# VojtaHavlicek/AlphaZero-Piskvorky

Hardware: AMD Instinct MI355X
Metric: mcts_node_expansions_per_sec (higher is better)
Workload: dtype f32; 1 GPU; 15x15 / 5-in-a-row self-play, 1024 concurrent games per GPU, 400 sims/move (BASELINE.json configs[3] per-GPU shard), GomokuNet random-init weights, numpy-compatible RNG tapes; board=15, win_length=5, sims_per_move=400, games_per_gpu=1024, engines_per_gpu=4, search_kernel=lock-step (k_trunk, k_fc, k_step per evaluation batch), parallelism=games sharded x1

## Files before the change

alphazero-piskvorky_amd/_capi.py:

```python
import ctypes as C
import os
import subprocess

import numpy as np

_HERE = os.path.dirname(os.path.abspath(__file__))
LIB_PATH = os.environ.get("AZ_ENGINE_LIB") or os.path.join(_HERE, "libaz_engine.so")

STATE_DICT_ORDER = [
    "conv1.weight", "conv1.bias", "conv2.weight", "conv2.bias", "conv3.weight", "conv3.bias",
    "policy_conv.weight", "policy_conv.bias", "policy_fc.weight", "policy_fc.bias",
    "value_conv.weight", "value_conv.bias", "value_fc1.weight", "value_fc1.bias",
    "value_fc2.weight", "value_fc2.bias",
]

AZ_EVAL_NET, AZ_EVAL_SYNTHETIC = 0, 1
AZ_RES_NONE, AZ_RES_X, AZ_RES_O, AZ_RES_DRAW = 0, 1, 2, 3
AZ_AUG_NONE, AZ_AUG_REFERENCE4, AZ_AUG_DIHEDRAL8 = 1, 4, 8
AZ_MODEL_PLAIN, AZ_MODEL_RESNET = 0, 1
AZ_TRUNK_F32, AZ_TRUNK_BF16X3, AZ_TRUNK_F16X2 = 0, 1, 2
AZ_MAX_SIMULATIONS, AZ_DEEP_MAX_SIMULATIONS = 1024, 65534
REUSE_MAX_SIMULATIONS = 1023

EXPORTS = [
    "az_create", "az_create_deep", "az_destroy", "az_last_error", "az_load_weights", "az_load_weights_resnet", "az_net_eval", "az_search", "az_search_batch", "az_search_callback", "az_selfplay",
    "az_selfplay_begin", "az_selfplay_step", "az_selfplay_end", "az_selfplay_games", "az_selfplay_records", "az_selfplay_clear", "az_record_bytes", "az_selfplay_pack", "az_examples_from_packed",
    "az_examples_gather", "az_arena", "az_rules_replay", "az_rng_selfplay_tape", "az_rng_uniforms", "az_set_profiling", "az_set_subtree_reuse", "az_get_counters", "az_get_lanes", "az_get_persistent", "az_set_virtual_loss", "az_set_eval_cache",
    "az_set_trunk_mode", "az_get_trunk_mode", "az_set_leaf_symmetry", "az_emul_split",
    "az_set_start_positions", "az_get_start_positions",
    "az_set_resign", "az_get_resign", "az_selfplay_values", "az_selfplay_pack_values", "az_selfplay_resign_info",
    "az_resign_mix", "az_resign_exempt",
    "az_set_playout_cap", "az_get_playout_cap", "az_playout_cap_full", "az_selfplay_sims", "az_selfplay_export_count",
    "az_set_forced_playouts", "az_get_forced_playouts", "az_forced_prune",
    "az_set_selection", "az_get_selection", "az_selection_tables",
    "az_set_candidates", "az_get_candidates", "az_candidate_mask",
    "az_set_gumbel", "az_get_gumbel", "az_gumbel_schedule", "az_gumbel_target", "az_gumbel_vmix", "az_rng_selfplay_tape_gumbel",
    "az_set_external_evaluator", "az_get_external_evaluator", "az_ext_capacity", "az_ext_stats",
    "az_set_solver", "az_get_solver", "az_last_proof", "az_selfplay_proofs", "az_solver_counts", "az_solver_stops",
    "az_set_win_rule", "az_get_win_rule", "az_rules_winner",
    "az_set_threat_search", "az_get_threat_search", "az_threat_batch", "az_threat_solve", "az_selfplay_threats", "az_threat_stats",
    "az_set_rng", "az_get_rng", "az_rng_philox4x32", "az_rng_log", "az_rng_exp", "az_rng_philox_tape", "az_rng_philox_tape_device",
    "az_set_delta_eval", "az_get_delta_eval", "az_delta_max_tiles", "az_delta_stats", "az_net_eval_delta", "az_delta_lists", "az_delta_lists_full",
    "az_dist_unique_id", "az_dist_init", "az_dist_rank", "az_dist_world", "az_dist_counts", "az_dist_gather_records",
    "az_dist_allreduce_sum", "az_dist_broadcast",
]
AZ_DIST_ID_BYTES = 128


class AzError(RuntimeError):
    pass


class az_config(C.Structure):
    _fields_ = [("board_size", C.c_int32), ("win_length", C.c_int32), ("num_simulations", C.c_int32),
                ("slots", C.c_int32), ("c_puct", C.c_double), ("dirichlet_alpha", C.c_double),
                ("dirichlet_weight", C.c_double), ("eval_kind", C.c_int32), ("device", C.c_int32),
                ("log_table", C.POINTER(C.c_float)), ("model", C.c_int32), ("engines", C.c_int32)]


class az_selfplay_args(C.Structure):
    _fields_ = [("seed0", C.c_uint64), ("num_games", C.c_int32), ("max_plies", C.c_int32),
                ("temperature_table", C.POINTER(C.c_double)), ("noise_tape", C.POINTER(C.c_double)),
                ("u_tape", C.POINTER(C.c_double)), ("tape_stride", C.c_int64)]


class az_counters(C.Structure):
    _fields_ = [("games", C.c_int64), ("plies", C.c_int64), ("records", C.c_int64), ("simulations", C.c_int64),
                ("expansions", C.c_int64), ("root_evals", C.c_int64), ("terminal_hits", C.c_int64),
                ("depth_sum", C.c_int64), ("steps", C.c_int64), ("seconds", C.c_double), ("nn_seconds", C.c_double),
                ("trunk_seconds", C.c_double), ("trunk_launches", C.c_int64), ("trunk_boards", C.c_int64),
                ("step_seconds", C.c_double), ("duplicate_leaves", C.c_int64), ("cache_lookups", C.c_int64),
                ("cache_hits", C.c_int64), ("tape_wait_seconds", C.c_double), ("tape_threads", C.c_int64),
                ("host_cpus", C.c_int64)]

    def as_dict(self):
# ... 104 lines not shown
            L.az_rng_selfplay_tape_gumbel.argtypes = [C.c_uint64, C.c_int, C.c_int, C.c_void_p, C.c_void_p]
        if hasattr(L, "az_set_external_evaluator"):
            L.az_set_external_evaluator.argtypes = [C.c_void_p, C.POINTER(az_ext_evaluator)]
            L.az_get_external_evaluator.argtypes = [C.c_void_p]
            L.az_ext_capacity.argtypes = [C.c_void_p]
            L.az_ext_stats.argtypes = [C.c_void_p, C.POINTER(C.c_int64), C.POINTER(C.c_int64)]
        if hasattr(L, "az_set_solver"):
            L.az_set_solver.argtypes = [C.c_void_p, C.c_int]
            L.az_get_solver.argtypes = [C.c_void_p]
            L.az_last_proof.argtypes = [C.c_void_p, C.c_int, C.c_void_p, C.c_void_p, C.POINTER(C.c_int32)]
            L.az_solver_stops.argtypes = [C.c_void_p, C.POINTER(C.c_int64)]
            L.az_selfplay_proofs.argtypes = [C.c_void_p, C.c_void_p]
            L.az_solver_counts.argtypes = [C.c_int, C.c_void_p, C.c_void_p, C.c_void_p]
        if hasattr(L, "az_set_win_rule"):
            L.az_set_win_rule.argtypes = [C.c_void_p, C.c_int]
            L.az_get_win_rule.argtypes = [C.c_void_p]
            L.az_rules_winner.argtypes = [C.c_void_p, C.c_int, C.c_int, C.c_int]
        if hasattr(L, "az_set_threat_search"):
            L.az_set_threat_search.argtypes = [C.c_void_p, C.c_int, C.c_int]
            L.az_get_threat_search.argtypes = [C.c_void_p, C.POINTER(C.c_int), C.POINTER(C.c_int)]
            L.az_threat_batch.argtypes = [C.c_void_p, C.c_int, C.c_void_p, C.c_void_p, C.c_int, C.c_int] + [C.c_void_p] * 5
            L.az_threat_solve.argtypes = [C.c_void_p, C.c_int, C.c_int, C.c_int, C.c_int, C.c_int, C.c_int] + [C.c_void_p] * 4
            L.az_selfplay_threats.argtypes = [C.c_void_p, C.c_void_p]
            L.az_threat_stats.argtypes = [C.c_void_p] + [C.POINTER(C.c_int64)] * 5
        if hasattr(L, "az_set_delta_eval"):
            L.az_set_delta_eval.argtypes = [C.c_void_p, C.c_int]
            L.az_get_delta_eval.argtypes = [C.c_void_p]
            L.az_delta_max_tiles.argtypes = [C.c_void_p, C.c_int]
            L.az_delta_stats.argtypes = [C.c_void_p] + [C.POINTER(C.c_int64)] * 4 + [C.c_void_p]
            L.az_net_eval_delta.argtypes = [C.c_void_p, C.c_int, C.c_void_p, C.c_int, C.c_int] + [C.c_void_p] * 7
            L.az_delta_lists.argtypes = [C.c_int, C.c_int] + [C.c_void_p] * 5
        if hasattr(L, "az_delta_lists_full"):
            L.az_delta_lists_full.argtypes = [C.c_int] + [C.c_void_p] * 4
        if hasattr(L, "az_set_rng"):
            L.az_set_rng.argtypes = [C.c_void_p, C.c_int]
            L.az_get_rng.argtypes = [C.c_void_p]
            L.az_rng_philox4x32.argtypes = [C.c_void_p, C.c_void_p, C.c_void_p]
            L.az_rng_philox4x32.restype = None
            L.az_rng_log.argtypes = L.az_rng_exp.argtypes = [C.c_double]
            L.az_rng_log.restype = L.az_rng_exp.restype = C.c_double
            L.az_rng_philox_tape.argtypes = [C.c_uint64, C.c_int, C.c_double, C.c_int, C.c_int, C.c_void_p, C.c_void_p]
            L.az_rng_philox_tape_device.argtypes = [C.c_void_p, C.c_uint64, C.c_int, C.c_double, C.c_int, C.c_int, C.c_void_p, C.c_void_p]
        _LIB = L
    return _LIB


def _p(a):
    return None if a is None else a.ctypes.data_as(C.c_void_p)


def _dp(a):
    return None if a is None else a.ctypes.data_as(C.POINTER(C.c_double))


def rng_selfplay_tape(seed, n, alpha=0.3, max_plies=0):
    nn = n * n
    plies = max_plies if 0 < max_plies < nn else nn
    total = sum(nn - m for m in range(plies))
    noise = np.zeros(total, np.float64)
    u = np.zeros(nn, np.float64)
    rc = lib().az_rng_selfplay_tape(int(seed), n, float(alpha), int(max_plies), _p(noise), _p(u))
    if rc:
        raise AzError(f"az_rng_selfplay_tape failed ({rc})")
    return noise, u[:plies]


# ... 865 lines not shown
```

alphazero-piskvorky_amd/csrc/az_delta.h:

```cpp
#pragma once
#include "az_net.h"

constexpr int DELTA_MAX_CHANGED = 8;
constexpr int DELTA_TILES_DEFAULT = 12;
constexpr int DELTA_CNT = 4 + 16;

template <int N>
struct DeltaGeo : NetGeo<N> {
    typedef NetGeo<N> B;
    static constexpr int IMG = 96 * B::CS;
    static constexpr int STRIDE = IMG + B::FROW;
    static constexpr int MAXM = ((B::nn + 15) / 16) * 16;
    static constexpr int C3 = 4;
};

__host__ __device__ inline int delta_dist(int n, int pr, int pc, const unsigned char *changed, int nch)
{
    int best = 255;
    for (int i = 0; i < nch; i++) {
        const int cr = changed[i] / n, cc = changed[i] - cr * n;
        const int dr = pr - 1 - cr < 0 ? cr - (pr - 1) : pr - 1 - cr, dc = pc - 1 - cc < 0 ? cc - (pc - 1) : pc - 1 - cc;
        const int dd = dr > dc ? dr : dc;
        best = dd < best ? dd : best;
    }
    return best;
}
__host__ __device__ inline bool delta_member(int n, int list, int pr, int pc, int dist)
{
    const bool inb = pr >= 1 && pr <= n && pc >= 1 && pc <= n;
    return list < 3 ? (inb && dist <= list + 1) : dist <= list;
}
template <int N>
struct DeltaLists {
    typedef DeltaGeo<N> G;
    unsigned short wpos[3][G::MAXM], cell[3][G::MAXM];
    unsigned short halo[2][G::PP];
    int cnt[5];
    __host__ __device__ int tiles(int l) const { return (cnt[l] + 15) >> 4; }
    __host__ __device__ void put(int list, int at, int pr, int pc)
    {
        const unsigned short pos = (unsigned short)(pr * G::PW + pc);
        if (list < 3) { wpos[list][at] = pos; cell[list][at] = (unsigned short)((pr - 1) * N + (pc - 1)); }
        else halo[list - 3][at] = pos;
    }
    __host__ __device__ void junk(int list, int i)
    {
        const int c = cnt[list], at = c + i;
        if (c > 0 && at < tiles(list) * 16) { wpos[list][at] = wpos[list][c - 1]; cell[list][at] = 0xFFFF; }
    }
};
template <int N>
__host__ __device__ inline void delta_lists_serial(const unsigned char *changed, int nch, DeltaLists<N> &L)
{
    typedef DeltaGeo<N> G;
    for (int l = 0; l < 5; l++) L.cnt[l] = 0;
    for (int p = 0; p < G::PP; p++) {
        const int pr = p / G::PW, pc = p - pr * G::PW;
        const int dist = delta_dist(N, pr, pc, changed, nch);
        for (int l = 0; l < 5; l++)
            if (delta_member(N, l, pr, pc, dist)) L.put(l, L.cnt[l]++, pr, pc);
    }
    for (int l = 0; l < 3; l++)
        for (int i = 0; i < 16; i++) L.junk(l, i);
}
template <int N>
__host__ __device__ inline void delta_full_put(DeltaLists<N> &L, int pr, int pc)
{
    if (pr < 1 || pr > N || pc < 1 || pc > N) return;
    for (int l = 0; l < 3; l++) L.put(l, (pr - 1) * N + (pc - 1), pr, pc);
}
template <int N>
__host__ __device__ inline void delta_full_cnt(DeltaLists<N> &L, int l) { L.cnt[l] = l < 3 ? N * N : 0; }
template <int N>
__host__ __device__ inline void delta_lists_full(DeltaLists<N> &L)
{
    typedef DeltaGeo<N> G;
    for (int p = 0; p < G::PP; p++) delta_full_put<N>(L, p / G::PW, p % G::PW);
    for (int l = 0; l < 5; l++) delta_full_cnt<N>(L, l);
    for (int l = 0; l < 3; l++)
        for (int i = 0; i < 16; i++) L.junk(l, i);
}

#ifdef __HIPCC__
#ifdef AZ_STAMPS
#define AZ_DSTAMP(k) do { if (threadIdx.x == 0 && dbg) dbg[(size_t)blockIdx.x * 16 + (k)] = __builtin_amdgcn_s_memtime(); } while (0)
#define AZ_DSTAMP_VAL(k, v) do { if (threadIdx.x == 0 && dbg) dbg[(size_t)blockIdx.x * 16 + (k)] = (unsigned long long)(v); } while (0)
#else
#define AZ_DSTAMP(k) do { } while (0)
#define AZ_DSTAMP_VAL(k, v) do { } while (0)
#endif

template <class G>
__device__ __forceinline__ void delta_heads(const NetWeights &w, float *__restrict__ frow, const float *out3, const float *hdq_lds,
                                            const unsigned short *cellof, int ncell, int wave, int lane)
{
    if (wave * 32 >= ncell) return;
    const int half = (lane >> 2) & 1;
    const int m = wave * 32 + (lane >> 3) * 4 + (lane & 3);
    float hb[4];
#pragma unroll
    for (int i = 0; i < 4; i++) hb[i] = (half * 4 + i) < 6 ? w.hdb[half * 4 + i] : 0.0f;
    const float4 *ap = reinterpret_cast<const float4 *>(hdq_lds) + (lane & 7);
    const float4 *bp = reinterpret_cast<const float4 *>(out3 + (m < ncell ? m : 0) * OUT3_CM_STRIDE);
    f32x4 acc = f32x4{0.f, 0.f, 0.f, 0.f};
#pragma unroll
    for (int k4 = 0; k4 < 32; k4++) {
        const float4 a = ap[k4 * 8], b = bp[k4];
        acc = __builtin_amdgcn_mfma_f32_4x4x1f32(a.x, b.x, acc, 0, 0, 0);
        acc = __builtin_amdgcn_mfma_f32_4x4x1f32(a.y, b.y, acc, 0, 0, 0);
        acc = __builtin_amdgcn_mfma_f32_4x4x1f32(a.z, b.z, acc, 0, 0, 0);
        acc = __builtin_amdgcn_mfma_f32_4x4x1f32(a.w, b.w, acc, 0, 0, 0);
    }
    if (m < ncell) {
        const int cell = cellof[m];
        if (cell != 0xFFFF) {
#pragma unroll
// ... 54 lines not shown
        float4 *z = reinterpret_cast<float4 *>(lds);
        for (int i = tid; i < (96 * G::CS) / 4; i += G::NW * 64) z[i] = float4{0.f, 0.f, 0.f, 0.f};
    }
    __syncthreads();
    float *inA = lds, *inB = lds + 32 * G::CS;
    if (e_me) inB[e_pos] = 1.0f;
    if (e_op) inB[G::CS + e_pos] = 1.0f;
    __syncthreads();
    conv_layer<G, 4, 32, CONV_OUT_PACKED>(inB, inA, w.c1, w.c1b, wpos, cellof, wave, lane);
    __syncthreads();
    for (int i = tid; i < 3 * G::CS; i += G::NW * 64) inB[i] = 0.0f;
    __syncthreads();
    conv_layer<G, 32, 64, CONV_OUT_PACKED>(inA, inB, w.c2, w.c2b, wpos, cellof, wave, lane);
    __syncthreads();
    float *row = base + ((size_t)b * 2 + par) * DG::STRIDE;
    {
        const float4 *s = reinterpret_cast<const float4 *>(lds);
        float4 *g = reinterpret_cast<float4 *>(row);
        for (int i = tid; i < DG::IMG / 4; i += G::NW * 64) g[i] = s[i];
    }
    conv_layer<G, 64, 128, CONV_OUT3_CM>(inB, lds, w.c3, w.c3b, wpos, cellof, wave, lane);
    __syncthreads();
    trunk_heads<G>(d, w, net_id, row + DG::IMG - (size_t)b * G::FROW, lds, hdq_lds, cellof, b, wave, lane);
    if (tid == 0 && par == 0) cnt[(size_t)b * DELTA_CNT + 3] += 2ull;
}

template <int N>
__global__ __launch_bounds__(NetGeo<N>::NW * 64) void k_trunk_delta(DevState d, NetWeights w, int net_id, float *__restrict__ feat,
                                                                     const float *__restrict__ base, unsigned char *done,
                                                                     unsigned long long *cnt, int max_tiles, unsigned long long *dbg)
{
    typedef DeltaGeo<N> G;
    constexpr int NT = G::NW * 64;
    static_assert(G::G == 1 && NT >= G::PP && NT == 512, "one board per workgroup, one thread per padded position");
    static_assert(G::C3 * 16 * OUT3_CM_STRIDE <= 32 * G::CS, "a chunk's conv3 image fits the dead conv1 image");
    static_assert(G::STRIDE % 4 == 0, "16-byte rows");
    __shared__ __attribute__((aligned(16))) float lds[G::IMG];
    __shared__ __attribute__((aligned(16))) float planes[4 * G::CS];
    __shared__ __attribute__((aligned(16))) float hdq_lds[1024];
    __shared__ DeltaLists<N> L;
    __shared__ unsigned char changed[DELTA_MAX_CHANGED];
    __shared__ int s_nch;
    __shared__ int s_wc[5][5];
    const int b = blockIdx.x;
    if (b >= d.B) return;
    const int tid = threadIdx.x, lane = tid & 63;
    const int wave = __builtin_amdgcn_readfirstlane(tid >> 6);
    AZ_DSTAMP(0);
    AZ_DSTAMP_VAL(14, __builtin_amdgcn_s_memrealtime());
#ifdef AZ_STAMPS
    for (int k = 1; k < 14; k++) AZ_DSTAMP_VAL(k, 0);
#endif
    {
        const int kind = d.leaf_kind[b];
        if (!((kind == LEAF_ROOT || kind == LEAF_EXPAND) && d.s_status[b] == SLOT_ACTIVE && d.s_net[b] == net_id)) {
            if (tid == 0) done[b] = 1;
            return;
        }
    }
    const float2 hq = reinterpret_cast<const float2 *>(w.hdq)[tid];
    const u64 *lf = d.leaf + (size_t)b * 8, *bd = d.board + (size_t)b * 8;
    const int last = d.leaf_last[b];
    int stones = 0;
#pragma unroll
    for (int i = 0; i < 8; i++) stones += __popcll(lf[i]) - __popcll(bd[i]);
    const int par = stones & 1;
    bool e_me = false, e_op = false, e_last = false;
    int e_pos = G::PW + 1;
    if (tid == 0) s_nch = 0;
    for (int i = tid; i < 4 * G::CS; i += NT) planes[i] = 0.0f;
    reinterpret_cast<float2 *>(hdq_lds)[tid] = hq;
    __syncthreads();
    if (tid < G::nn) {
        const int r = tid / N, c = tid - r * N;
        e_pos = (r + 1) * G::PW + (c + 1);
        e_me = (lf[tid >> 6] >> (tid & 63)) & 1ull;
        e_op = (lf[4 + (tid >> 6)] >> (tid & 63)) & 1ull;
        e_last = last == tid;
        const bool x = (bd[tid >> 6] >> (tid & 63)) & 1ull, o = (bd[4 + (tid >> 6)] >> (tid & 63)) & 1ull;
        const bool me_is_x = (d.s_player[b] == 1) != (par == 1);
        if (e_me != (me_is_x ? x : o) || e_op != (me_is_x ? o : x) || e_last) {
            const int k = atomicAdd(&s_nch, 1);
            if (k < DELTA_MAX_CHANGED) changed[k] = (unsigned char)tid;
        }
        if (e_me) planes[e_pos] = 1.0f;
        if (e_op) planes[G::CS + e_pos] = 1.0f;
        if (e_last) planes[2 * G::CS + e_pos] = 1.0f;
    }
    __syncthreads();
    const int nch = s_nch;
    bool full = nch > DELTA_MAX_CHANGED;
    const int pr = tid / G::PW, pc = tid - pr * G::PW;
    int dist = 255;
    if (!full) {
        u64 bal[5] = {0, 0, 0, 0, 0};
        if (wave < 5) {
            const bool in_img = tid < G::PP;
            if (in_img) dist = delta_dist(N, pr, pc, changed, nch);
#pragma unroll
            for (int l = 0; l < 5; l++) {
                bal[l] = __ballot(in_img && delta_member(N, l, pr, pc, dist));
                if (lane == 0) s_wc[wave][l] = __popcll(bal[l]);
            }
        }
        __syncthreads();
        if (wave < 5 && tid < G::PP) {
#pragma unroll
            for (int l = 0; l < 5; l++) {
                if (!((bal[l] >> lane) & 1ull)) continue;
                int at = __popcll(bal[l] & ((1ull << lane) - 1ull));
                for (int v = 0; v < wave; v++) at += s_wc[v][l];
                L.put(l, at, pr, pc);
            }
        }
        if (tid < 5) L.cnt[tid] = s_wc[0][tid] + s_wc[1][tid] + s_wc[2][tid] + s_wc[3][tid] + s_wc[4][tid];
        __syncthreads();
        full = L.tiles(2) > max_tiles;
        if (full) __syncthreads();
    }
    float *inA = lds, *inB = lds + 32 * G::CS;
    if (full) {
        if (tid < G::PP) delta_full_put<N>(L, pr, pc);
        if (tid < 5) delta_full_cnt<N>(L, tid);
        float4 *z = reinterpret_cast<float4 *>(lds);
        for (int i = tid; i < G::IMG / 4; i += NT) z[i] = float4{0.f, 0.f, 0.f, 0.f};
        __syncthreads();
    }
    const int t1 = L.tiles(0), t2 = L.tiles(1), t3 = L.tiles(2);
    AZ_DSTAMP(1);
    AZ_DSTAMP_VAL(13, t3);
    if (tid < 48) L.junk(tid >> 4, tid & 15);
    if (tid == 0) {
        if (full) { done[b] = 0; cnt[(size_t)b * DELTA_CNT + 1] += 1ull; }
        else {
            done[b] = (unsigned char)(1 + t3);
            cnt[(size_t)b * DELTA_CNT + 0] += 1ull;
            cnt[(size_t)b * DELTA_CNT + 2] += (unsigned long long)t3;
            cnt[(size_t)b * DELTA_CNT + 4 + t3] += 1ull;
        }
    }
    constexpr int WR = (G::PP + 63) / 64;
    static_assert(WR * 64 >= G::PP && G::NW == 8, "the rounds reach the longest list; one conv1 plane and two conv2 planes per wave");
    f32x4 w1[WR], w2[2][WR];
    float fr[6];
    f32x4 *l4 = reinterpret_cast<f32x4 *>(lds);
    float *frow = feat + (size_t)b * G::FROW;
    const bool keep = !full && tid < G::PP && delta_member(N, 2, pr, pc, 0) && dist > 3;
    const int fcell = (pr - 1) * N + (pc - 1);
    const int n3 = full ? 0 : L.cnt[3], n4 = full ? 0 : L.cnt[4];
    {
        const float *brow = base + ((size_t)b * 2 + par) * G::STRIDE;
        const f32x4 *g4 = reinterpret_cast<const f32x4 *>(brow);
        const float *bf = brow + G::IMG;
        delta_rounds<0, WR>([&](auto jc) {
            constexpr int j = decltype(jc)::value;
            if (j * 64 + lane < n3) w1[j] = g4[wave * G::CS + L.halo[0][j * 64 + lane]];
        });
        delta_rounds<0, WR>([&](auto jc) {
            constexpr int j = decltype(jc)::value;
            if (j * 64 + lane < n4) {
                const int pos = L.halo[1][j * 64 + lane];
                w2[0][j] = g4[(8 + wave) * G::CS + pos];
                w2[1][j] = g4[(16 + wave) * G::CS + pos];
            }
        });
        if (keep) {
#pragma unroll
            for (int i = 0; i < 6; i++) fr[i] = bf[i * G::nn + fcell];
        }
        delta_rounds<0, WR>([&](auto jc) {
            constexpr int j = decltype(jc)::value;
            if (j * 64 + lane < n3) l4[wave * G::CS + L.halo[0][j * 64 + lane]] = w1[j];
        });
    }
    __syncthreads();
    AZ_DSTAMP(2);
    for (int t0 = 0; t0 < t1; t0 += 4)
        conv_layer<G, 4, 32, CONV_OUT_PACKED, 4>(planes, inA, w.c1, w.c1b, L.wpos[0], L.cell[0], wave, lane, t0, t1 - t0 < 4 ? t1 - t0 : 4);
    delta_rounds<0, WR>([&](auto jc) {
        constexpr int j = decltype(jc)::value;
        if (j * 64 + lane < n4) {
            const int pos = L.halo[1][j * 64 + lane];
            l4[(8 + wave) * G::CS + pos] = w2[0][j];
            l4[(16 + wave) * G::CS + pos] = w2[1][j];
        }
    });
    if (keep) {
#pragma unroll
        for (int i = 0; i < 6; i++) frow[i * G::nn + fcell] = fr[i];
    }
    __syncthreads();
    AZ_DSTAMP(3);
    for (int t0 = 0; t0 < t2;) {
        const int c = t2 - t0;
        if (c > 2) { conv_layer<G, 32, 64, CONV_OUT_PACKED, 4>(inA, inB, w.c2, w.c2b, L.wpos[1], L.cell[1], wave, lane, t0, c < 4 ? c : 4); t0 += 4; }
        else { conv_layer<G, 32, 64, CONV_OUT_PACKED, 2>(inA, inB, w.c2, w.c2b, L.wpos[1], L.cell[1], wave, lane, t0, c); t0 += 2; }
    }
    __syncthreads();
    AZ_DSTAMP(4);
    for (int t0 = 0; t0 < t3; t0 += G::C3) {
        const int c = t3 - t0 < G::C3 ? t3 - t0 : G::C3;
        float *o3 = lds - t0 * 16 * OUT3_CM_STRIDE;
        if (c == 4) conv_layer<G, 64, 128, CONV_OUT3_CM, 4>(inB, o3, w.c3, w.c3b, L.wpos[2], L.cell[2], wave, lane, t0, 4);
        else if (c == 3) conv_layer<G, 64, 128, CONV_OUT3_CM, 3>(inB, o3, w.c3, w.c3b, L.wpos[2], L.cell[2], wave, lane, t0, 3);
        else if (c == 2) conv_layer<G, 64, 128, CONV_OUT3_CM, 2>(inB, o3, w.c3, w.c3b, L.wpos[2], L.cell[2], wave, lane, t0, 2);
        else conv_layer<G, 64, 128, CONV_OUT3_CM, 1>(inB, o3, w.c3, w.c3b, L.wpos[2], L.cell[2], wave, lane, t0, 1);
        __syncthreads();
        AZ_DSTAMP(5 + 2 * (t0 / G::C3));
        delta_heads<G>(w, frow, lds, hdq_lds, L.cell[2] + t0 * 16, c * 16, wave, lane);
        __syncthreads();
        AZ_DSTAMP(6 + 2 * (t0 / G::C3));
        AZ_DSTAMP_VAL(15, __builtin_amdgcn_s_memrealtime());
    }
}
#endif
```

alphazero-piskvorky_amd/csrc/az_engine.hip:

```cpp
#include <hip/hip_runtime.h>
#include <dlfcn.h>
#include <sched.h>

#include <algorithm>
#include <atomic>
#include <chrono>
#include <condition_variable>
#include <cmath>
#include <cstdarg>
#include <cstdio>
#include <cstdlib>
#include <cstring>
#include <mutex>
#include <string>
#include <thread>
#include <vector>

#define AZ_ENGINE_TU 1
#include "../../include/az_engine.h"
#include "az_launch.h"

#include "az_host.h"

static thread_local std::string g_create_error;
// ... 2434 lines not shown
}

extern "C" int az_delta_lists(int n, int count, const uint8_t *changed, uint16_t *wpos, uint16_t *cell, uint16_t *halo, int32_t *cnt)
{
    if (n != 15 || count < 0 || count > DELTA_MAX_CHANGED || (count && !changed) || !wpos || !cell || !halo || !cnt) return AZ_ERR_INVALID;
    for (int i = 0; i < count; i++) if (changed[i] >= 15 * 15) return AZ_ERR_INVALID;
    static DeltaLists<15> L;
    static std::mutex m;
    std::lock_guard<std::mutex> lock(m);
    memset(&L, 0xEE, sizeof L);
    delta_lists_serial<15>(changed, count, L);
    memcpy(wpos, L.wpos, sizeof L.wpos);
    memcpy(cell, L.cell, sizeof L.cell);
    memcpy(halo, L.halo, sizeof L.halo);
    for (int l = 0; l < 5; l++) cnt[l] = L.cnt[l];
    return AZ_OK;
}

extern "C" int az_delta_lists_full(int n, uint16_t *wpos, uint16_t *cell, uint16_t *halo, int32_t *cnt)
{
    if (n != 15 || !wpos || !cell || !halo || !cnt) return AZ_ERR_INVALID;
    static DeltaLists<15> L;
    static std::mutex m;
    std::lock_guard<std::mutex> lock(m);
    memset(&L, 0xEE, sizeof L);
    delta_lists_full<15>(L);
    memcpy(wpos, L.wpos, sizeof L.wpos);
    memcpy(cell, L.cell, sizeof L.cell);
    memcpy(halo, L.halo, sizeof L.halo);
    for (int l = 0; l < 5; l++) cnt[l] = L.cnt[l];
    return AZ_OK;
}

extern "C" int az_net_eval_delta(az_engine *e, int slot, const uint8_t *root, int root_player, int count, const uint8_t *boards,
                                 const uint8_t *players, const int16_t *lasts, float *logits, float *policy, float *value, int32_t *path)
{
    if (!e || slot < 0 || slot > 1 || count < 0 || !root || !boards || !players || !lasts || (root_player != 1 && root_player != 2))
        return fail(e, AZ_ERR_INVALID, "az_net_eval_delta: bad argument");
    if (!e->net[slot].loaded) return fail(e, AZ_ERR_NO_WEIGHTS, "weights slot %d not loaded", slot);
    if (e->run.open) return fail(e, AZ_ERR_STATE, "az_net_eval_delta: a self-play episode is open on this engine");
    if (!e->ops->trunk_delta || e->cfg.model != AZ_MODEL_PLAIN || e->cfg.eval_kind != AZ_EVAL_NET)
        return fail(e, AZ_ERR_INVALID, "az_net_eval_delta: no delta evaluation for this board size or net");
    DEVICE_GUARD(e);
    int rc = ensure_delta_buffers(e);
    if (rc) return rc;
    const Lane &L = e->lanes[0];
    const DeltaRoot dr{root, root_player, path};
    return eval_positions(e, "az_net_eval_delta", slot, count, boards, players, lasts, logits, policy, value, &dr, [&](LaunchCtx &lc, int) {
        lc.delta_base = (float *)L.delta_base.p;
        lc.delta_done = (unsigned char *)L.delta_done.p;
        lc.delta_cnt = (unsigned long long *)L.delta_cnt.p;
        lc.delta_tiles = e->delta_tiles;
        e->ops->trunk_base(lc, slot);
        e->ops->trunk_delta(lc, slot);
    });
}

extern "C" int az_selfplay_proofs(az_engine *e, int8_t *roots)
{
    if (!e || !e->have_episode) return fail(e, AZ_ERR_STATE, "no episode has been run");
    if (!roots) return fail(e, AZ_ERR_INVALID, "az_selfplay_proofs: null buffer");
    if (!e->episode_solver || !e->rec_proof.p) return fail(e, AZ_ERR_STATE, "az_selfplay_proofs: the episode ran without the solver");
    DEVICE_GUARD(e);
    return read_record_array(e, e->rec_proof, roots);
}

// ... 1012 lines not shown
```

include/az_engine.h:

```cpp
#ifndef AZ_ENGINE_H
#define AZ_ENGINE_H

#include <stdint.h>

#ifdef __cplusplus
extern "C" {
#endif

typedef struct az_engine az_engine;

typedef enum {
    AZ_OK = 0,
    AZ_ERR_INVALID = -1,
    AZ_ERR_NO_DEVICE = -2,
    AZ_ERR_HIP = -3,
    AZ_ERR_ILLEGAL_MOVE = -4,
    AZ_ERR_NO_WEIGHTS = -5,
    AZ_ERR_STATE = -6
} az_status;

enum { AZ_EVAL_NET = 0, AZ_EVAL_SYNTHETIC = 1 };
enum { AZ_RES_NONE = 0, AZ_RES_X = 1, AZ_RES_O = 2, AZ_RES_DRAW = 3 };
enum { AZ_AUG_REFERENCE4 = 4, AZ_AUG_DIHEDRAL8 = 8, AZ_AUG_NONE = 1 };
enum { AZ_TRUNK_F32 = 0, AZ_TRUNK_BF16X3 = 1, AZ_TRUNK_F16X2 = 2 };
// ... 132 lines not shown
             int32_t *nply);

int az_rules_replay(az_engine *e, int games, int max_len, const int16_t *actions, uint8_t *term_before, uint8_t *boards,
                    int32_t *players, int32_t *results, int32_t *first_illegal);

int az_rng_selfplay_tape(uint64_t seed, int board_size, double alpha, int max_plies, double *noise, double *u);
int az_rng_uniforms(uint64_t seed, int count, double *u);
int az_rng_selfplay_tape_gumbel(uint64_t seed, int board_size, int max_plies, double *noise, double *u);

enum { AZ_RNG_NUMPY = 0, AZ_RNG_PHILOX = 1 };
enum { AZ_TAPE_DIRICHLET = 0, AZ_TAPE_GUMBEL = 1 };
#define AZ_RNG_PHILOX_ATTEMPTS 64
int az_set_rng(az_engine *e, int mode);
int az_get_rng(const az_engine *e);
void az_rng_philox4x32(const uint32_t ctr[4], const uint32_t key[2], uint32_t out[4]);
double az_rng_log(double x);
double az_rng_exp(double x);
int az_rng_philox_tape(uint64_t seed, int board_size, double alpha, int max_plies, int kind, double *noise, double *u);
int az_rng_philox_tape_device(az_engine *e, uint64_t seed0, int games, double alpha, int max_plies, int kind, double *noise_out,
                              double *u_out);

int az_set_subtree_reuse(az_engine *e, int on);

int az_set_virtual_loss(az_engine *e, int leaves);

int az_set_eval_cache(az_engine *e, int64_t entries);

int az_set_delta_eval(az_engine *e, int on);
int az_get_delta_eval(const az_engine *e);
int az_delta_max_tiles(az_engine *e, int tiles);
int az_delta_stats(const az_engine *e, int64_t *delta, int64_t *full, int64_t *tiles, int64_t *base, int64_t *by_tiles);
int az_delta_lists(int n, int count, const uint8_t *changed, uint16_t *wpos, uint16_t *cell, uint16_t *halo, int32_t *cnt);
int az_delta_lists_full(int n, uint16_t *wpos, uint16_t *cell, uint16_t *halo, int32_t *cnt);
int az_net_eval_delta(az_engine *e, int slot, const uint8_t *root, int root_player, int count, const uint8_t *boards,
                      const uint8_t *players, const int16_t *lasts, float *logits, float *policy, float *value, int32_t *path);

int az_set_leaf_symmetry(az_engine *e, int on);

int az_set_start_positions(az_engine *e, int count, const uint8_t *boards ,
                           const uint8_t *players, const int16_t *lasts, int64_t first);
int az_get_start_positions(const az_engine *e);

enum { AZ_RULE_FREESTYLE = 0, AZ_RULE_EXACT = 1 };
int az_set_win_rule(az_engine *e, int rule);
int az_get_win_rule(const az_engine *e);
int az_rules_winner(const uint8_t *board, int n, int k, int rule);

uint32_t az_resign_mix(uint32_t x);
int az_resign_exempt(uint32_t key, int playout_permille);
int az_set_resign(az_engine *e, double threshold, int min_ply, int playout_permille);
int az_get_resign(const az_engine *e, double *threshold, int *min_ply, int *playout_permille);
int az_selfplay_values(az_engine *e, float *values);
int az_selfplay_pack_values(az_engine *e, float *values_dev);
int az_selfplay_resign_info(az_engine *e, int32_t *cross_ply, uint8_t *exempt);

int az_playout_cap_full(uint32_t key, int ply, int full_permille);
int az_set_playout_cap(az_engine *e, int fast_sims, int full_permille, int export_full_only);
int az_get_playout_cap(const az_engine *e, int *fast_sims, int *full_permille, int *export_full_only);
int az_selfplay_sims(az_engine *e, int32_t *sims);
int az_selfplay_export_count(az_engine *e, int64_t *records);

int az_set_forced_playouts(az_engine *e, double k, int prune);
int az_get_forced_playouts(const az_engine *e, double *k, int *prune);
int64_t az_forced_prune(double k, double c_puct, int count, const int32_t *visits, const double *W, const float *prior, int32_t *out);

int az_set_selection(az_engine *e, int on, double fpu, double fpu_root, double cpuct_base, double cpuct_factor);
// ... 49 lines not shown
```

Baseline: 6.606 million node-expansions/s.

## Restructure delta-eval kernel prologue to cut barriers and shared-memory atomics

The delta evaluation kernel now finds changed cells with wave-uniform bit arithmetic (readfirstlane plus per-lane popcount/ctz) instead of a shared-memory atomic scan. It also folds list counting into a single vectorized read of per-wave counts, which removes several __syncthreads. Conv1 now runs over the conv3 tile list instead of copying halo values, conv1/conv2 weights are prefetched before the early exit, and statistics counters use relaxed atomics. The goal is lower per-leaf prologue latency and less synchronisation. In exchange conv1 may compute more tiles, and the list-building logic is more intricate.

```diff
diff --git a/alphazero-piskvorky_amd/_capi.py b/alphazero-piskvorky_amd/_capi.py
--- a/alphazero-piskvorky_amd/_capi.py
+++ b/alphazero-piskvorky_amd/_capi.py
@@ -41,6 +41,7 @@
     "az_set_threat_search", "az_get_threat_search", "az_threat_batch", "az_threat_solve", "az_selfplay_threats", "az_threat_stats",
     "az_set_rng", "az_get_rng", "az_rng_philox4x32", "az_rng_log", "az_rng_exp", "az_rng_philox_tape", "az_rng_philox_tape_device",
     "az_set_delta_eval", "az_get_delta_eval", "az_delta_max_tiles", "az_delta_stats", "az_net_eval_delta", "az_delta_lists", "az_delta_lists_full",
+    "az_delta_changed",
     "az_dist_unique_id", "az_dist_init", "az_dist_rank", "az_dist_world", "az_dist_counts", "az_dist_gather_records",
     "az_dist_allreduce_sum", "az_dist_broadcast",
 ]
@@ -211,6 +212,8 @@
             L.az_delta_lists.argtypes = [C.c_int, C.c_int] + [C.c_void_p] * 5
         if hasattr(L, "az_delta_lists_full"):
             L.az_delta_lists_full.argtypes = [C.c_int] + [C.c_void_p] * 4
+        if hasattr(L, "az_delta_changed"):
+            L.az_delta_changed.argtypes = [C.c_int, C.c_void_p, C.c_void_p, C.c_int, C.c_int] + [C.c_void_p] * 3
         if hasattr(L, "az_set_rng"):
             L.az_set_rng.argtypes = [C.c_void_p, C.c_int]
             L.az_get_rng.argtypes = [C.c_void_p]
diff --git a/alphazero-piskvorky_amd/csrc/az_delta.h b/alphazero-piskvorky_amd/csrc/az_delta.h
--- a/alphazero-piskvorky_amd/csrc/az_delta.h
+++ b/alphazero-piskvorky_amd/csrc/az_delta.h
@@ -48,6 +48,11 @@
         const int c = cnt[list], at = c + i;
         if (c > 0 && at < tiles(list) * 16) { wpos[list][at] = wpos[list][c - 1]; cell[list][at] = 0xFFFF; }
     }
+    __host__ __device__ void junk_at(int list, int c, int i, int pos)
+    {
+        const int at = c + i;
+        if (i >= 0 && i < 16 && at < ((c + 15) >> 4) * 16) { wpos[list][at] = (unsigned short)pos; cell[list][at] = 0xFFFF; }
+    }
 };
 template <int N>
 __host__ __device__ inline void delta_lists_serial(const unsigned char *changed, int nch, DeltaLists<N> &L)
@@ -81,7 +86,47 @@
         for (int i = 0; i < 16; i++) L.junk(l, i);
 }
 
+template <int N>
+__host__ __device__ inline __attribute__((always_inline)) int delta_changed(const u64 *leaf, const u64 *board, int player, int last, int k, int *count, int *parity)
+{
+    static_assert(N * N > 192 && N * N <= 256, "four words of cells, the last one in part");
+    int stones = 0;
+#pragma unroll
+    for (int i = 0; i < 8; i++) stones += __builtin_popcountll(leaf[i]) - __builtin_popcountll(board[i]);
+    const int par = stones & 1;
+    const bool me_is_x = (player == 1) != (par == 1);
+    u64 v = 0;
+    int total = 0, wi = 0, kk = 0;
+#pragma unroll
+    for (int i = 0; i < 4; i++) {
+        const u64 bme = me_is_x ? board[i] : board[4 + i], bop = me_is_x ? board[4 + i] : board[i];
+        u64 dw = (leaf[i] ^ bme) | (leaf[4 + i] ^ bop);
+        if (last >= 0 && last < N * N && (last >> 6) == i) dw |= 1ull << (last & 63);
+        if (i == 3 && N * N < 256) dw &= (1ull << ((N * N) & 63)) - 1ull;
+        const int c = __builtin_popcountll(dw);
+        if (k >= total && k < total + c) { v = dw; wi = i; kk = k - total; }
+        total += c;
+    }
+#pragma unroll
+    for (int j = 0; j < DELTA_MAX_CHANGED - 1; j++)
+        if (j < kk) v &= v - 1ull;
+    *count = total;
+    *parity = par;
+    return (k >= 0 && k < total && k < DELTA_MAX_CHANGED && v) ? wi * 64 + __builtin_ctzll(v) : 0xFF;
+}
+
 #ifdef __HIPCC__
+__device__ __forceinline__ void delta_count(unsigned long long *p, unsigned long long v)
+{
+    (void)__hip_atomic_fetch_add(p, v, __ATOMIC_RELAXED, __HIP_MEMORY_SCOPE_AGENT);
+}
+
+__device__ __forceinline__ u64 delta_uniform(u64 v)
+{
+    const unsigned lo = __builtin_amdgcn_readfirstlane((unsigned)v), hi = __builtin_amdgcn_readfirstlane((unsigned)(v >> 32));
+    return ((u64)hi << 32) | lo;
+}
+
 #ifdef AZ_STAMPS
 #define AZ_DSTAMP(k) do { if (threadIdx.x == 0 && dbg) dbg[(size_t)blockIdx.x * 16 + (k)] = __builtin_amdgcn_s_memtime(); } while (0)
 #define AZ_DSTAMP_VAL(k, v) do { if (threadIdx.x == 0 && dbg) dbg[(size_t)blockIdx.x * 16 + (k)] = (unsigned long long)(v); } while (0)
@@ -202,16 +247,14 @@
 {
     typedef DeltaGeo<N> G;
     constexpr int NT = G::NW * 64;
-    static_assert(G::G == 1 && NT >= G::PP && NT == 512, "one board per workgroup, one thread per padded position");
+    static_assert(G::G == 1 && NT >= G::CS && NT == 512, "one board per workgroup, one thread per padded position");
     static_assert(G::C3 * 16 * OUT3_CM_STRIDE <= 32 * G::CS, "a chunk's conv3 image fits the dead conv1 image");
     static_assert(G::STRIDE % 4 == 0, "16-byte rows");
     __shared__ __attribute__((aligned(16))) float lds[G::IMG];
     __shared__ __attribute__((aligned(16))) float planes[4 * G::CS];
     __shared__ __attribute__((aligned(16))) float hdq_lds[1024];
     __shared__ DeltaLists<N> L;
-    __shared__ unsigned char changed[DELTA_MAX_CHANGED];
-    __shared__ int s_nch;
-    __shared__ int s_wc[5][5];
+    __shared__ __attribute__((aligned(16))) int s_wc[5][4];
     const int b = blockIdx.x;
     if (b >= d.B) return;
     const int tid = threadIdx.x, lane = tid & 63;
@@ -221,111 +264,113 @@
 #ifdef AZ_STAMPS
     for (int k = 1; k < 14; k++) AZ_DSTAMP_VAL(k, 0);
 #endif
-    {
-        const int kind = d.leaf_kind[b];
-        if (!((kind == LEAF_ROOT || kind == LEAF_EXPAND) && d.s_status[b] == SLOT_ACTIVE && d.s_net[b] == net_id)) {
-            if (tid == 0) done[b] = 1;
-            return;
-        }
-    }
+    const int kind = d.leaf_kind[b], status = d.s_status[b], snet = d.s_net[b], last = d.leaf_last[b], player = d.s_player[b];
+    u64 lf[8], bd[8];
+#pragma unroll
+    for (int i = 0; i < 8; i++) { lf[i] = delta_uniform(d.leaf[(size_t)b * 8 + i]); bd[i] = delta_uniform(d.board[(size_t)b * 8 + i]); }
     const float2 hq = reinterpret_cast<const float2 *>(w.hdq)[tid];
-    const u64 *lf = d.leaf + (size_t)b * 8, *bd = d.board + (size_t)b * 8;
-    const int last = d.leaf_last[b];
-    int stones = 0;
-#pragma unroll
-    for (int i = 0; i < 8; i++) stones += __popcll(lf[i]) - __popcll(bd[i]);
-    const int par = stones & 1;
-    bool e_me = false, e_op = false, e_last = false;
-    int e_pos = G::PW + 1;
-    if (tid == 0) s_nch = 0;
-    for (int i = tid; i < 4 * G::CS; i += NT) planes[i] = 0.0f;
-    reinterpret_cast<float2 *>(hdq_lds)[tid] = hq;
-    __syncthreads();
-    if (tid < G::nn) {
-        const int r = tid / N, c = tid - r * N;
-        e_pos = (r + 1) * G::PW + (c + 1);
-        e_me = (lf[tid >> 6] >> (tid & 63)) & 1ull;
-        e_op = (lf[4 + (tid >> 6)] >> (tid & 63)) & 1ull;
-        e_last = last == tid;
-        const bool x = (bd[tid >> 6] >> (tid & 63)) & 1ull, o = (bd[4 + (tid >> 6)] >> (tid & 63)) & 1ull;
-        const bool me_is_x = (d.s_player[b] == 1) != (par == 1);
-        if (e_me != (me_is_x ? x : o) || e_op != (me_is_x ? o : x) || e_last) {
-            const int k = atomicAdd(&s_nch, 1);
-            if (k < DELTA_MAX_CHANGED) changed[k] = (unsigned char)tid;
-        }
-        if (e_me) planes[e_pos] = 1.0f;
-        if (e_op) planes[G::CS + e_pos] = 1.0f;
-        if (e_last) planes[2 * G::CS + e_pos] = 1.0f;
-    }
-    __syncthreads();
-    const int nch = s_nch;
+    const ConvPre<4> pre1 = conv_prefetch<G, 4, 32>(w.c1, wave, lane);
+    if (!((kind == LEAF_ROOT || kind == LEAF_EXPAND) && status == SLOT_ACTIVE && snet == net_id)) {
+        if (tid == 0) done[b] = 1;
+        return;
+    }
+    int ch[DELTA_MAX_CHANGED], par, nch;
+    {
+        const int mine = delta_changed<N>(lf, bd, player, last, lane & (DELTA_MAX_CHANGED - 1), &nch, &par);
+#pragma unroll
+        for (int i = 0; i < DELTA_MAX_CHANGED; i++) ch[i] = __builtin_amdgcn_readlane(mine, i);
+    }
     bool full = nch > DELTA_MAX_CHANGED;
     const int pr = tid / G::PW, pc = tid - pr * G::PW;
+    const bool in_img = tid < G::PP, inb = in_img && pr >= 1 && pr <= N && pc >= 1 && pc <= N;
+    const int fcell = (pr - 1) * N + (pc - 1);
+    f32x4 *l4 = reinterpret_cast<f32x4 *>(lds);
+    if (tid < G::CS) {
+        const int cp = inb ? fcell : 0, wi = cp >> 6;
+        const u64 me = wi == 0 ? lf[0] : wi == 1 ? lf[1] : wi == 2 ? lf[2] : lf[3];
+        const u64 op = wi == 0 ? lf[4] : wi == 1 ? lf[5] : wi == 2 ? lf[6] : lf[7];
+        planes[tid] = inb && ((me >> (cp & 63)) & 1ull) ? 1.0f : 0.0f;
+        planes[G::CS + tid] = inb && ((op >> (cp & 63)) & 1ull) ? 1.0f : 0.0f;
+        planes[2 * G::CS + tid] = inb && last == cp ? 1.0f : 0.0f;
+        planes[3 * G::CS + tid] = 0.0f;
+    }
     int dist = 255;
+    u64 bal[4] = {0, 0, 0, 0};
+    if (!full && wave < 5) {
+        if (in_img) {
+#pragma unroll
+            for (int i = 0; i < DELTA_MAX_CHANGED; i++) {
+                if (i < nch) {
+                    const int cr = ch[i] / N, cc = ch[i] - cr * N;
+                    const int dr = pr - 1 - cr < 0 ? cr - (pr - 1) : pr - 1 - cr, dc = pc - 1 - cc < 0 ? cc - (pc - 1) : pc - 1 - cc;
+                    const int dd = dr > dc ? dr : dc;
+                    dist = dd < dist ? dd : dist;
+                }
+            }
+        }
+#pragma unroll
+        for (int l = 0; l < 4; l++) {
+            bal[l] = __ballot(in_img && delta_member(N, l < 3 ? l : 4, pr, pc, dist));
+            if (lane == 0) s_wc[wave][l] = __popcll(bal[l]);
+        }
+        if (in_img && !inb && dist <= 3) {
+#pragma unroll
+            for (int k = 0; k < 8; k++) l4[k * G::CS + tid] = f32x4{0.f, 0.f, 0.f, 0.f};
+        }
+    }
+    __syncthreads();
+    int c[4] = {G::nn, G::nn, G::nn, 0}, front[4] = {0, 0, 0, 0};
     if (!full) {
-        u64 bal[5] = {0, 0, 0, 0, 0};
-        if (wave < 5) {
-            const bool in_img = tid < G::PP;
-            if (in_img) dist = delta_dist(N, pr, pc, changed, nch);
-#pragma unroll
-            for (int l = 0; l < 5; l++) {
-                bal[l] = __ballot(in_img && delta_member(N, l, pr, pc, dist));
-                if (lane == 0) s_wc[wave][l] = __popcll(bal[l]);
+        c[0] = c[1] = c[2] = 0;
+#pragma unroll
+        for (int v = 0; v < 5; v++) {
+            const int4 r = reinterpret_cast<const int4 *>(&s_wc[0][0])[v];
+            const int rv[4] = {r.x, r.y, r.z, r.w};
+#pragma unroll
+            for (int l = 0; l < 4; l++) { c[l] += rv[l]; front[l] += v < wave ? rv[l] : 0; }
+        }
+        full = ((c[2] + 15) >> 4) > max_tiles;
+        if (full) { c[0] = c[1] = c[2] = G::nn; c[3] = 0; }
+    }
+    if (!full) {
+        if (wave < 5 && in_img) {
+#pragma unroll
+            for (int l = 0; l < 4; l++) {
+                if ((bal[l] >> lane) & 1ull) L.put(l < 3 ? l : 4, front[l] + __popcll(bal[l] & ((1ull << lane) - 1ull)), pr, pc);
+                if (l < 3 && bal[l] && front[l] + __popcll(bal[l]) == c[l])
+                    L.junk_at(l, c[l], lane, wave * 64 + 63 - __builtin_clzll(bal[l]));
             }
         }
-        __syncthreads();
-        if (wave < 5 && tid < G::PP) {
-#pragma unroll
-            for (int l = 0; l < 5; l++) {
-                if (!((bal[l] >> lane) & 1ull)) continue;
-                int at = __popcll(bal[l] & ((1ull << lane) - 1ull));
-                for (int v = 0; v < wave; v++) at += s_wc[v][l];
-                L.put(l, at, pr, pc);
-            }
-        }
-        if (tid < 5) L.cnt[tid] = s_wc[0][tid] + s_wc[1][tid] + s_wc[2][tid] + s_wc[3][tid] + s_wc[4][tid];
-        __syncthreads();
-        full = L.tiles(2) > max_tiles;
-        if (full) __syncthreads();
-    }
-    float *inA = lds, *inB = lds + 32 * G::CS;
-    if (full) {
-        if (tid < G::PP) delta_full_put<N>(L, pr, pc);
-        if (tid < 5) delta_full_cnt<N>(L, tid);
-        float4 *z = reinterpret_cast<float4 *>(lds);
-        for (int i = tid; i < G::IMG / 4; i += NT) z[i] = float4{0.f, 0.f, 0.f, 0.f};
-        __syncthreads();
-    }
-    const int t1 = L.tiles(0), t2 = L.tiles(1), t3 = L.tiles(2);
+    } else {
+        if (in_img) delta_full_put<N>(L, pr, pc);
+#pragma unroll
+        for (int l = 0; l < 3; l++) L.junk_at(l, G::nn, tid, N * G::PW + N);
+        for (int i = tid; i < G::IMG / 4; i += NT) l4[i] = f32x4{0.f, 0.f, 0.f, 0.f};
+    }
+    __syncthreads();
+    const int t2 = (c[1] + 15) >> 4, t3 = (c[2] + 15) >> 4, n4 = c[3];
     AZ_DSTAMP(1);
-    AZ_DSTAMP_VAL(13, t3);
-    if (tid < 48) L.junk(tid >> 4, tid & 15);
+    AZ_DSTAMP_VAL(13, t3 | (t2 << 8));
     if (tid == 0) {
-        if (full) { done[b] = 0; cnt[(size_t)b * DELTA_CNT + 1] += 1ull; }
+        unsigned long long *cb = cnt + (size_t)b * DELTA_CNT;
+        if (full) { done[b] = 0; delta_count(cb + 1, 1ull); }
         else {
             done[b] = (unsigned char)(1 + t3);
-            cnt[(size_t)b * DELTA_CNT + 0] += 1ull;
-            cnt[(size_t)b * DELTA_CNT + 2] += (unsigned long long)t3;
-            cnt[(size_t)b * DELTA_CNT + 4 + t3] += 1ull;
+            delta_count(cb + 0, 1ull);
+            delta_count(cb + 2, (unsigned long long)t3);
+            delta_count(cb + 4 + t3, 1ull);
         }
     }
     constexpr int WR = (G::PP + 63) / 64;
-    static_assert(WR * 64 >= G::PP && G::NW == 8, "the rounds reach the longest list; one conv1 plane and two conv2 planes per wave");
-    f32x4 w1[WR], w2[2][WR];
+    static_assert(WR * 64 >= G::PP && G::NW == 8, "the rounds reach the longest list; two conv2 planes per wave");
+    f32x4 w2[2][WR];
     float fr[6];
-    f32x4 *l4 = reinterpret_cast<f32x4 *>(lds);
     float *frow = feat + (size_t)b * G::FROW;
-    const bool keep = !full && tid < G::PP && delta_member(N, 2, pr, pc, 0) && dist > 3;
-    const int fcell = (pr - 1) * N + (pc - 1);
-    const int n3 = full ? 0 : L.cnt[3], n4 = full ? 0 : L.cnt[4];
+    const bool keep = !full && inb && dist > 3;
     {
         const float *brow = base + ((size_t)b * 2 + par) * G::STRIDE;
         const f32x4 *g4 = reinterpret_cast<const f32x4 *>(brow);
         const float *bf = brow + G::IMG;
-        delta_rounds<0, WR>([&](auto jc) {
-            constexpr int j = decltype(jc)::value;
-            if (j * 64 + lane < n3) w1[j] = g4[wave * G::CS + L.halo[0][j * 64 + lane]];
-        });
         delta_rounds<0, WR>([&](auto jc) {
             constexpr int j = decltype(jc)::value;
             if (j * 64 + lane < n4) {
@@ -338,15 +383,14 @@
 #pragma unroll
             for (int i = 0; i < 6; i++) fr[i] = bf[i * G::nn + fcell];
         }
-        delta_rounds<0, WR>([&](auto jc) {
-            constexpr int j = decltype(jc)::value;
-            if (j * 64 + lane < n3) l4[wave * G::CS + L.halo[0][j * 64 + lane]] = w1[j];
-        });
-    }
-    __syncthreads();
+    }
+    const ConvPre<32> pre2 = conv_prefetch<G, 32, 64>(w.c2, wave, lane);
     AZ_DSTAMP(2);
-    for (int t0 = 0; t0 < t1; t0 += 4)
-        conv_layer<G, 4, 32, CONV_OUT_PACKED, 4>(planes, inA, w.c1, w.c1b, L.wpos[0], L.cell[0], wave, lane, t0, t1 - t0 < 4 ? t1 - t0 : 4);
+    float *inA = lds, *inB = lds + 32 * G::CS;
+    for (int t0 = 0; t0 < t3; t0 += 4)
+        conv_layer<G, 4, 32, CONV_OUT_PACKED, 4>(planes, inA, w.c1, w.c1b, L.wpos[2], L.cell[2], wave, lane, t0, t3 - t0 < 4 ? t3 - t0 : 4,
+                                                 0, nullptr, nullptr, &pre1);
+    reinterpret_cast<float2 *>(hdq_lds)[tid] = hq;
     delta_rounds<0, WR>([&](auto jc) {
         constexpr int j = decltype(jc)::value;
         if (j * 64 + lane < n4) {
@@ -361,23 +405,25 @@
     }
     __syncthreads();
     AZ_DSTAMP(3);
-    for (int t0 = 0; t0 < t2;) {
-        const int c = t2 - t0;
-        if (c > 2) { conv_layer<G, 32, 64, CONV_OUT_PACKED, 4>(inA, inB, w.c2, w.c2b, L.wpos[1], L.cell[1], wave, lane, t0, c < 4 ? c : 4); t0 += 4; }
-        else { conv_layer<G, 32, 64, CONV_OUT_PACKED, 2>(inA, inB, w.c2, w.c2b, L.wpos[1], L.cell[1], wave, lane, t0, c); t0 += 2; }
+    for (int t0 = 0; t0 < t2; t0 += 4) {
+        const int c2 = t2 - t0 < 4 ? t2 - t0 : 4;
+        if (c2 == 4) conv_layer<G, 32, 64, CONV_OUT_PACKED, 4>(inA, inB, w.c2, w.c2b, L.wpos[1], L.cell[1], wave, lane, t0, 4, 0, nullptr, nullptr, &pre2);
+        else if (c2 == 3) conv_layer<G, 32, 64, CONV_OUT_PACKED, 3>(inA, inB, w.c2, w.c2b, L.wpos[1], L.cell[1], wave, lane, t0, 3, 0, nullptr, nullptr, &pre2);
+        else if (c2 == 2) conv_layer<G, 32, 64, CONV_OUT_PACKED, 2>(inA, inB, w.c2, w.c2b, L.wpos[1], L.cell[1], wave, lane, t0, 2, 0, nullptr, nullptr, &pre2);
+        else conv_layer<G, 32, 64, CONV_OUT_PACKED, 1>(inA, inB, w.c2, w.c2b, L.wpos[1], L.cell[1], wave, lane, t0, 1, 0, nullptr, nullptr, &pre2);
     }
     __syncthreads();
     AZ_DSTAMP(4);
     for (int t0 = 0; t0 < t3; t0 += G::C3) {
-        const int c = t3 - t0 < G::C3 ? t3 - t0 : G::C3;
+        const int c3 = t3 - t0 < G::C3 ? t3 - t0 : G::C3;
         float *o3 = lds - t0 * 16 * OUT3_CM_STRIDE;
-        if (c == 4) conv_layer<G, 64, 128, CONV_OUT3_CM, 4>(inB, o3, w.c3, w.c3b, L.wpos[2], L.cell[2], wave, lane, t0, 4);
-        else if (c == 3) conv_layer<G, 64, 128, CONV_OUT3_CM, 3>(inB, o3, w.c3, w.c3b, L.wpos[2], L.cell[2], wave, lane, t0, 3);
-        else if (c == 2) conv_layer<G, 64, 128, CONV_OUT3_CM, 2>(inB, o3, w.c3, w.c3b, L.wpos[2], L.cell[2], wave, lane, t0, 2);
+        if (c3 == 4) conv_layer<G, 64, 128, CONV_OUT3_CM, 4>(inB, o3, w.c3, w.c3b, L.wpos[2], L.cell[2], wave, lane, t0, 4);
+        else if (c3 == 3) conv_layer<G, 64, 128, CONV_OUT3_CM, 3>(inB, o3, w.c3, w.c3b, L.wpos[2], L.cell[2], wave, lane, t0, 3);
+        else if (c3 == 2) conv_layer<G, 64, 128, CONV_OUT3_CM, 2>(inB, o3, w.c3, w.c3b, L.wpos[2], L.cell[2], wave, lane, t0, 2);
         else conv_layer<G, 64, 128, CONV_OUT3_CM, 1>(inB, o3, w.c3, w.c3b, L.wpos[2], L.cell[2], wave, lane, t0, 1);
         __syncthreads();
         AZ_DSTAMP(5 + 2 * (t0 / G::C3));
-        delta_heads<G>(w, frow, lds, hdq_lds, L.cell[2] + t0 * 16, c * 16, wave, lane);
+        delta_heads<G>(w, frow, lds, hdq_lds, L.cell[2] + t0 * 16, c3 * 16, wave, lane);
         __syncthreads();
         AZ_DSTAMP(6 + 2 * (t0 / G::C3));
         AZ_DSTAMP_VAL(15, __builtin_amdgcn_s_memrealtime());
diff --git a/alphazero-piskvorky_amd/csrc/az_engine.hip b/alphazero-piskvorky_amd/csrc/az_engine.hip
--- a/alphazero-piskvorky_amd/csrc/az_engine.hip
+++ b/alphazero-piskvorky_amd/csrc/az_engine.hip
@@ -2490,6 +2490,20 @@
     return AZ_OK;
 }
 
+extern "C" int az_delta_changed(int n, const uint64_t *leaf, const uint64_t *board, int player, int last, uint8_t *changed,
+                                int32_t *count, int32_t *parity)
+{
+    if (n != 15 || !leaf || !board || !changed || !count || !parity || (player != 1 && player != 2) || last < -1 || last >= 15 * 15)
+        return AZ_ERR_INVALID;
+    u64 lf[8], bd[8];
+    for (int i = 0; i < 8; i++) { lf[i] = leaf[i]; bd[i] = board[i]; }
+    int par = 0, cnt = 0;
+    for (int k = 0; k < DELTA_MAX_CHANGED; k++) changed[k] = (uint8_t)delta_changed<15>(lf, bd, player, last, k, &cnt, &par);
+    *count = cnt;
+    *parity = par;
+    return AZ_OK;
+}
+
 extern "C" int az_net_eval_delta(az_engine *e, int slot, const uint8_t *root, int root_player, int count, const uint8_t *boards,
                                  const uint8_t *players, const int16_t *lasts, float *logits, float *policy, float *value, int32_t *path)
 {
diff --git a/include/az_engine.h b/include/az_engine.h
--- a/include/az_engine.h
+++ b/include/az_engine.h
@@ -188,6 +188,8 @@
 int az_delta_stats(const az_engine *e, int64_t *delta, int64_t *full, int64_t *tiles, int64_t *base, int64_t *by_tiles);
 int az_delta_lists(int n, int count, const uint8_t *changed, uint16_t *wpos, uint16_t *cell, uint16_t *halo, int32_t *cnt);
 int az_delta_lists_full(int n, uint16_t *wpos, uint16_t *cell, uint16_t *halo, int32_t *cnt);
+int az_delta_changed(int n, const uint64_t *leaf, const uint64_t *board, int player, int last, uint8_t *changed,
+                     int32_t *count, int32_t *parity);
 int az_net_eval_delta(az_engine *e, int slot, const uint8_t *root, int root_player, int count, const uint8_t *boards,
                       const uint8_t *players, const int16_t *lasts, float *logits, float *policy, float *value, int32_t *path);
 
```

After: 6.959 million node-expansions/s (median of 6 runs). 5.3% higher.
